# ShreyasBhaktharam/RDEIC

Hardware: AMD Instinct MI355X
Metric: 512x512 images/sec encode+relay-decode @ fixed bpp; 1/2/4/8 GPU (higher is better)
Workload: dtype bf16; 1 GPU; config 2: global batch 16 (16/GPU) 512x512, 2-step relay DDIM, encode+entropy-code+decode+VAE-decode; global_batch=16, image_size=512, ddim_steps=2, sampler=ddim, parallelism=dp1, codec_sessions_per_gpu=5

## Files before the change

include/rdeic_hip.h:

```cpp
#ifndef RDEIC_HIP_H
#define RDEIC_HIP_H
#include <stddef.h>
#include <stdint.h>
#ifdef __cplusplus
extern "C" {
#endif

int rdeic_version(void);
int rdeic_abi_count(void);

typedef struct rdeic_conv_desc {
  const void* in0;
  const void* in1;
  int32_t c0, c1;
  int32_t ld0, ld1;
  int32_t n, h, w;
  int32_t up2;
  const void* weight;
  int32_t wld;
  const float* bias;
  int32_t cout, kh, kw, stride, pad_t, pad_l;
  int32_t ho, wo;
  const float* gn_ab;
  int32_t gn_silu;
  const float* emb;
  int32_t emb_ld;
  int32_t act;
  float act_param;
  const void* res;
  int32_t res_ld;
  void* out;
  int32_t out_ld;
  int32_t out_mode;
  int32_t dtype;
  int32_t out_f32;
  int32_t batch;
  int64_t in_bs, w_bs, out_bs;
  float* gn_part;
  int32_t gn_hw;
  int32_t reserved;
  const float* ln_rows;
  const float* ln_colsum;
} rdeic_conv_desc;

int rdeic_conv2d(const rdeic_conv_desc* d, void* stream);
int rdeic_conv2d_tile(const rdeic_conv_desc* d, int32_t tile, void* stream);
int rdeic_conv2d_splitk(const rdeic_conv_desc* d, int32_t splits, float* ws, size_t ws_floats, void* stream);
int rdeic_conv2d_up2_phases(const rdeic_conv_desc* d, int64_t phase_stride, int32_t tile, void* stream);
int rdeic_conv2d_up2_group(const rdeic_conv_desc* d);
int rdeic_set_conv_path(int32_t path);
int rdeic_set_conv_option(int32_t key, int32_t value);

size_t rdeic_groupnorm_ws_floats(int32_t n, int32_t hw, int32_t c);
size_t rdeic_groupnorm_parts_floats(int64_t rows, int32_t c, int32_t hw);
int rdeic_groupnorm_parts_ab(const float* p0, int32_t c0, const float* p1, int32_t c1, int32_t n, int32_t hw,
// ... 104 lines not shown
#define RDEIC_PROF_GN_STATS 3
#define RDEIC_PROF_GN_APPLY 4
#define RDEIC_PROF_GEMM 5
#define RDEIC_PROF_ATTN_D512 6
#define RDEIC_PROF_CONV_BYTES 7
int rdeic_prof_start(int32_t capacity, int32_t every);
int rdeic_prof_read_keys(int32_t kind, int64_t* keys, int64_t* launches, double* work, double* ms, int32_t cap);
#define RDEIC_COUNT_HALO_CONV 0
#define RDEIC_COUNT_GN_APPLY 1
#define RDEIC_COUNT_LAYERNORM 2
#define RDEIC_COUNT_HALO_SMALL 3
#define RDEIC_COUNT_LN_FUSED 4
#define RDEIC_COUNT_SPLITK 5
#define RDEIC_COUNT_EDGE 6
#define RDEIC_COUNT_GN_PARTS_APPLY 7
#define RDEIC_COUNT_KINDS 8
int64_t rdeic_launch_count(int32_t kind);
int rdeic_layernorm_rowstats(const void* x, int32_t rows, int32_t c, int32_t ld, float eps, float* ms,
                             void* stream);
int rdeic_launch_count_reset(void);
int rdeic_prof_stop(void);
int rdeic_prof_read(int32_t kind, int64_t* launches, double* work, double* ms);

typedef struct rdeic_gemm_desc {
  const void* a;
  int64_t a_bs1, a_bs2, a_sm, a_sk;
  const void* b;
  int64_t b_bs1, b_bs2, b_sk, b_sn;
  void* c;
  int64_t c_bs1, c_bs2, c_sm;
  int32_t batch, nb2, m, n, k, ksplit, dtype, c_f32;
// ... 94 lines not shown
```

rdeic_amd/_lib.py:

```python
from __future__ import annotations

import ctypes as C
import os
import threading

_HERE = os.path.dirname(os.path.abspath(__file__))
LIB_PATH = os.environ.get("RDEIC_LIB") or os.path.join(_HERE, "lib", "librdeic_hip.so")

EINVAL, ENOSPC, EBADMSG, ELAUNCH = -22, -28, -74, -5
_ERRNAMES = {EINVAL: "EINVAL (bad argument/shape)", ENOSPC: "ENOSPC (output capacity)",
             EBADMSG: "EBADMSG (corrupt or truncated bitstream)", ELAUNCH: "kernel launch failure"}


class RdeicError(RuntimeError):
    def __init__(self, fn: str, code: int):
        super().__init__(f"{fn} failed: {code} {_ERRNAMES.get(code, '')}")
        self.code = code


class BitstreamError(RdeicError, ValueError):
    """Corrupt / truncated bitstream (the reference's 'decode failure')."""


class ConvDesc(C.Structure):
# ... 1 lines not shown
        ("in0", C.c_void_p), ("in1", C.c_void_p),
        ("c0", C.c_int32), ("c1", C.c_int32), ("ld0", C.c_int32), ("ld1", C.c_int32),
        ("n", C.c_int32), ("h", C.c_int32), ("w", C.c_int32), ("up2", C.c_int32),
        ("weight", C.c_void_p), ("wld", C.c_int32),
        ("bias", C.c_void_p),
        ("cout", C.c_int32), ("kh", C.c_int32), ("kw", C.c_int32), ("stride", C.c_int32),
        ("pad_t", C.c_int32), ("pad_l", C.c_int32),
        ("ho", C.c_int32), ("wo", C.c_int32),
        ("gn_ab", C.c_void_p), ("gn_silu", C.c_int32),
        ("emb", C.c_void_p), ("emb_ld", C.c_int32),
        ("act", C.c_int32), ("act_param", C.c_float),
        ("res", C.c_void_p), ("res_ld", C.c_int32),
        ("out", C.c_void_p), ("out_ld", C.c_int32), ("out_mode", C.c_int32),
        ("dtype", C.c_int32), ("out_f32", C.c_int32),
        ("batch", C.c_int32), ("in_bs", C.c_int64), ("w_bs", C.c_int64), ("out_bs", C.c_int64),
        ("gn_part", C.c_void_p), ("gn_hw", C.c_int32), ("reserved", C.c_int32),
        ("ln_rows", C.c_void_p), ("ln_colsum", C.c_void_p),
    ]


class GemmDesc(C.Structure):
    _fields_ = [
        ("a", C.c_void_p), ("a_bs1", C.c_int64), ("a_bs2", C.c_int64), ("a_sm", C.c_int64), ("a_sk", C.c_int64),
        ("b", C.c_void_p), ("b_bs1", C.c_int64), ("b_bs2", C.c_int64), ("b_sk", C.c_int64), ("b_sn", C.c_int64),
        ("c", C.c_void_p), ("c_bs1", C.c_int64), ("c_bs2", C.c_int64), ("c_sm", C.c_int64),
        ("batch", C.c_int32), ("nb2", C.c_int32), ("m", C.c_int32), ("n", C.c_int32), ("k", C.c_int32),
        ("ksplit", C.c_int32), ("dtype", C.c_int32), ("c_f32", C.c_int32),
        ("alpha", C.c_float), ("beta", C.c_float), ("rsum", C.c_void_p), ("rsum_bs", C.c_int64),
    ]


# ... 170 lines not shown
```

rdeic_amd/csrc/conv_common.h:

```cpp
#pragma once
#include "common.h"
#include "../../include/rdeic_hip.h"
#include "prof.h"

namespace rdeic_conv {

struct ConvArgs {
  const char* in0; const char* in1;
  int c0, c1, ld0, ld1;
  int n, h, w, up2;
  const char* weight; int wld;
  const float* bias;
  int cout, kh, kw, stride, pad_t, pad_l, ho, wo;
  const float* gn_ab; int gn_silu;
  const float* emb; int emb_ld;
  int act; float act_param;
  const char* res; int res_ld;
  char* out; int out_ld, out_mode;
  int out_f32;
  int M, cin, ktot, nk;
  long in_bs, w_bs, out_bs;
  int batch;
  int epi_vec;
  int splits, kper;
  float* gn_part;
  int gn_row0;
  int gn_hw;
  const float* ln_rows;
  const float* ln_cs;
};

__device__ __forceinline__ float ln_fold(const ConvArgs& a, int m, int n, float v) {
  const float2 ms = reinterpret_cast<const float2*>(a.ln_rows)[m];
  return ms.y * (v - ms.x * a.ln_cs[n]);
}

constexpr int ROWB = 144;

template <typename T, bool SWZ = true> __host__ __device__ constexpr int tile_rowb() { return (sizeof(T) == 2 && SWZ) ? 128 : ROWB; }
template <typename T, bool SWZ = true> __device__ __forceinline__ int chunk_key(int r) {
  if constexpr (sizeof(T) == 2 && SWZ) return (((r >> 3) & 1) << 1) | (((r >> 1) & 1) << 2);
  return 0;
}
template <typename T, int BM, int BN, bool SWZ = true> __host__ __device__ constexpr int conv_lds_bytes() {
// ... 395 lines not shown
      for (int h = 0; h < 2; ++h)
#pragma unroll
        for (int e = 0; e < 4; e += 2) {
          const f32x2 xv = {to_f32(from_f32<bf16>(v[8 * h + e])), to_f32(from_f32<bf16>(v[8 * h + e + 1]))};
          const f32x2 gt = {to_f32(from_f32<bf16>(v[8 * h + 4 + e])), to_f32(from_f32<bf16>(v[8 * h + 5 + e]))};
          const f32x2 r = xv * gelu_fast2(gt);
          gv[4 * h + e] = from_f32<bf16>(r.x);
          gv[4 * h + e + 1] = from_f32<bf16>(r.y);
        }
      *reinterpret_cast<uint4*>(reinterpret_cast<bf16*>(a.out) + (long)m * a.out_ld + (nn >> 1)) =
          *reinterpret_cast<uint4*>(gv);
    }
  }
}

constexpr unsigned kOOB = 0x80000000u;

template <int N>
__device__ __forceinline__ void wait_vm() {
  asm volatile("s_waitcnt vmcnt(%0)" ::"n"(N) : "memory");
}

__device__ __forceinline__ int dma_key(int r) { return (((r >> 3) & 1) << 1) | (((r >> 1) & 1) << 2); }

typedef __attribute__((address_space(3))) void* lds_ptr_t;

__device__ __forceinline__ void dma16(__amdgpu_buffer_rsrc_t rs, char* lds_dst, unsigned voff, int soff) {
  __builtin_amdgcn_raw_ptr_buffer_load_lds(rs, (lds_ptr_t)lds_dst, 16, (int)voff, soff, 0, 0);
}

// ... 8 lines not shown
#endif

__device__ __forceinline__ void wait_vm_rt(int n) {
  switch (n) {
    case 0: wait_vm<0>(); break;
    case 1: wait_vm<1>(); break;
    case 2: wait_vm<2>(); break;
    case 3: wait_vm<3>(); break;
    case 4: wait_vm<4>(); break;
    case 5: wait_vm<5>(); break;
    case 6: wait_vm<6>(); break;
    default: wait_vm<7>(); break;
  }
}

extern int g_conv_path, g_epi_vec, g_swz, g_force_tile, g_dma, g_halo, g_halo8, g_edge, g_up2_phases;

int make_args(const rdeic_conv_desc* d, ConvArgs& a, bool& vec);
bool dma_ok(const rdeic_conv_desc* d, const ConvArgs& a, unsigned& b0, unsigned& b1, unsigned& bw);
int launch_dma_auto(const ConvArgs& a, unsigned b0, unsigned b1, unsigned bw, hipStream_t s, int tile,
                    int gn_hw = 0, bool* fused = nullptr);
int dma_grouped(const rdeic_conv_desc* d, int tile, hipStream_t s, bool* fused = nullptr);
bool halo_ok(const rdeic_conv_desc* d, const ConvArgs& a);
int launch_halo(const rdeic_conv_desc* d, ConvArgs a, hipStream_t s, bool* fused);
int launch_edge(const rdeic_conv_desc* d, const ConvArgs& a, hipStream_t s, bool* fused);
int up2_phase_group(const rdeic_conv_desc* d);
bool up2_phases_ok(const rdeic_conv_desc* d, long phase_stride);
int launch_up2_phases(const rdeic_conv_desc* d, long phase_stride, int tile, hipStream_t s, bool* fused);
}
```

rdeic_amd/csrc/conv_dma.hip:

```cpp
#include "conv_common.h"

namespace rdeic_conv {

template <int TM, int TN, int WTM, int WTN, class PixMap = PixSame>
__device__ __forceinline__ void epilogue_scalar(const f32x4 (&acc)[TM][TN], const ConvArgs& a, int m0, int n0, int wm,
                                                int wn, int lane, PixMap pmap = PixMap{}) {
  if (a.out_mode == 2) return;
  const int lrow = lane & 15, lq = lane >> 4;
  const int hw_o = a.ho * a.wo;
  const bool of32 = a.out_f32;
#pragma unroll
  for (int i = 0; i < TM; ++i) {
#pragma unroll
    for (int r = 0; r < 4; ++r) {
      const int m = m0 + wm * WTM + i * 16 + lq * 4 + r;
      if (m >= a.M) continue;
      const int img = m / hw_o;
      int oy = 0, ox = 0;
      if (a.out_mode == 1) { const int rem = m - img * hw_o; oy = rem / a.wo; ox = rem - oy * a.wo; }
#pragma unroll
      for (int j = 0; j < TN; ++j) {
        const int nn = n0 + wn * WTN + j * 16 + lrow;
        if (nn >= a.cout) continue;
        float v = acc[i][j][r];
// ... 7 lines not shown
          const long p = ((long)img * (2 * a.ho) + (2 * oy + dy)) * (2 * a.wo) + (2 * ox + dx);
          oidx = p * a.out_ld + c;
          ridx = p * a.res_ld + c;
        } else {
          oidx = pmap(m) * a.out_ld + nn;
          ridx = pmap(m) * a.res_ld + nn;
        }
        if (a.res) v += of32 ? reinterpret_cast<const float*>(a.res)[ridx] : to_f32(reinterpret_cast<const bf16*>(a.res)[ridx]);
        if (of32) reinterpret_cast<float*>(a.out)[oidx] = v;
        else reinterpret_cast<bf16*>(a.out)[oidx] = from_f32<bf16>(v);
      }
    }
  }
}

template <int BM, int BN, int WGM, int WGN, int S, int EP, bool GEG = false, bool PH = false>
__device__ __forceinline__ void conv_dma_body(ConvArgs a, int tiles_n, unsigned bytes0, unsigned bytes1,
                                              unsigned bytesw) {
  constexpr int KB = 64;
  constexpr int NW = WGM * WGN, NT = NW * 64;
  constexpr int RB = KB * 2;
  constexpr int RPI = 1024 / RB;
  constexpr int LPR = RB / 16;
  constexpr int KSUB = KB / 32;
  constexpr int A_BYTES = BM * RB, STAGE = (BM + BN) * RB;
  constexpr int AI = BM / NW / RPI, BI = BN / NW / RPI;
  constexpr int PER = AI + BI;
  constexpr int WTM = BM / WGM, WTN = BN / WGN;
  constexpr int TM = WTM / 16, TN = WTN / 16;
  static_assert(AI >= 1 && BI >= 1 && AI * RPI * NW == BM && BI * RPI * NW == BN, "tile / wave split");
  static_assert(S >= 2 && S <= 4 && PER * (S - 2) <= 63, "ring");
// ... 159 lines not shown
  HALO_STAMP(2);
  if constexpr (PH) {
    const PixPhase pm{a.h, a.w, phase >> 1, phase & 1};
    if constexpr (TM % EP == 0 && (BM / EP) * (BN + 4) * 4 <= S * STAGE) {
      if (a.epi_vec && epi_vec_ok(a)) {
        epilogue_vec<BM, BN, WGM, WGN, NT, EP, RowsFrom, false, PixPhase>(acc, a, m0, n0, wm, wn, lane, tid, lds,
                                                                          RowsFrom{m0}, pm);
        HALO_STAMP(3);
        return;
      }
    }
    epilogue_scalar<TM, TN, WTM, WTN, PixPhase>(acc, a, m0, n0, wm, wn, lane, pm);
    HALO_STAMP(3);
    return;
  }
  if constexpr (TM % EP == 0 && (BM / EP) * (BN + 4) * 4 <= S * STAGE) {
    if ((a.epi_vec || a.out_mode == 2) && epi_vec_ok(a)) {
      if constexpr (GEG) epilogue_geglu<BM, BN, WGM, WGN, NT, EP>(acc, a, m0, n0, wm, wn, lane, tid, lds);
      else epilogue_vec<BM, BN, WGM, WGN, NT, EP>(acc, a, m0, n0, wm, wn, lane, tid, lds);
      HALO_STAMP(3);
      return;
    }
  }
  epilogue_scalar<TM, TN, WTM, WTN>(acc, a, m0, n0, wm, wn, lane);
  HALO_STAMP(3);
}

template <int BM, int BN, int WGM, int WGN, int S, int EP, bool GEG = false, bool PH = false>
__global__ __launch_bounds__(WGM * WGN * 64) void conv_dma_kernel(ConvArgs a, int tiles_n, unsigned bytes0,
                                                                  unsigned bytes1, unsigned bytesw) {
  conv_dma_body<BM, BN, WGM, WGN, S, EP, GEG, PH>(a, tiles_n, bytes0, bytes1, bytesw);
}

template <int BM, int BN, int WGM, int WGN, int S, int EP, bool GEG = false>
__global__ __launch_bounds__(WGM * WGN * 64) __attribute__((amdgpu_num_sgpr(80))) void conv_dma_kernel_2pc(
    ConvArgs a, int tiles_n, unsigned bytes0, unsigned bytes1, unsigned bytesw) {
  conv_dma_body<BM, BN, WGM, WGN, S, EP, GEG>(a, tiles_n, bytes0, bytes1, bytesw);
}

bool dma_ok(const rdeic_conv_desc* d, const ConvArgs& a, unsigned& b0, unsigned& b1, unsigned& bw) {
  if (d->dtype != 1 || d->gn_ab || (d->c0 % 64) || (d->c1 % 64) || (d->ld0 % 8) || ((uintptr_t)d->in0 % 16)) return false;
  if (d->c1 && ((d->ld1 % 8) || ((uintptr_t)d->in1 % 16))) return false;
  if (d->wld % 64 || a.ktot % 64) return false;
  const long pix = (long)d->n * d->h * d->w;
  const long e0 = ((pix - 1) * d->ld0 + d->c0) * 2 + (a.batch - 1) * d->in_bs * 2;
  const long e1 = d->c1 ? ((pix - 1) * d->ld1 + d->c1) * 2 : 16;
  const long ew = (long)d->cout * d->wld * 2 + (a.batch - 1) * d->w_bs * 2;
  if (e0 >= (1l << 31) || e1 >= (1l << 31) || ew >= (1l << 31)) return false;
  if (a.batch > 1 && (d->in_bs % 8 || d->w_bs % 8)) return false;
// ... 11 lines not shown
  return fits && (a.epi_vec || a.out_mode == 2) && epi_vec_ok(a);
}

template <int BM, int BN, int WGM, int WGN, int S, int EP>
int launch_dma(ConvArgs a, unsigned b0, unsigned b1, unsigned bw, hipStream_t s, int gn_hw, bool* fused) {
  if (a.gn_part) {
    const bool ok = a.splits <= 1 && a.batch == 1 && a.out_mode == 0 && gn_hw > 0 && gn_hw % 64 == 0 &&
                    stats_tile_ok<BM, BN, WGM, WGM * WGN * 64, EP>() && dma_vec_epilogue<BM, BN, WGM, WGN, S, EP>(a);
    if (!ok) a.gn_part = nullptr;
    if (fused) *fused = ok;
  }
  const int tn = cdiv(a.cout, BN);
  const long tiles = (long)cdiv(a.M, BM) * tn;
  dim3 grid((unsigned)tiles, 1, a.splits > 1 ? a.splits : a.batch);
  constexpr int lds = S * (BM + BN) * 128;
  const bool geg = a.out_mode == 2 && a.cout % 16 == 0 && a.out_ld % 8 == 0 && ((uintptr_t)a.out % 16) == 0 &&
                   dma_vec_epilogue<BM, BN, WGM, WGN, S, EP>(a);
  if constexpr (WGM * WGN == 16 && lds <= 80 * 1024) {
    hipLaunchKernelGGL((conv_dma_kernel_2pc<BM, BN, WGM, WGN, S, EP>), grid, dim3(WGM * WGN * 64), lds, s, a, tn, b0,
                       b1, bw);
  } else {
    if (geg)
      hipLaunchKernelGGL((conv_dma_kernel<BM, BN, WGM, WGN, S, EP, true>), grid, dim3(WGM * WGN * 64), lds, s, a, tn,
                         b0, b1, bw);
    else
      hipLaunchKernelGGL((conv_dma_kernel<BM, BN, WGM, WGN, S, EP>), grid, dim3(WGM * WGN * 64), lds, s, a, tn, b0, b1,
                         bw);
  }
  return launch_status();
}
}

int launch_dma_auto(const ConvArgs& a, unsigned b0, unsigned b1, unsigned bw, hipStream_t s, int tile, int gn_hw,
                    bool* fused) {
  if (tile < 21 || tile > 38) {
    const long zb = a.splits > 1 ? a.splits : a.batch;
    const long t128 = (long)cdiv(a.M, 128) * cdiv(a.cout, 128) * zb;
    const long t256 = (long)cdiv(a.M, 256) * cdiv(a.cout, 256) * zb;
// ... 56 lines not shown
  return RDEIC_OK;
}

namespace {
template <int BM, int BN, int WGM, int WGN, int S, int EP>
int launch_dma_ph(ConvArgs a, unsigned b0, unsigned b1, unsigned bw, hipStream_t s, bool* fused) {
  if (a.gn_part) {
    const bool ok = (a.h * a.w) % 64 == 0 && stats_tile_ok<BM, BN, WGM, WGM * WGN * 64, EP>() &&
                    dma_vec_epilogue<BM, BN, WGM, WGN, S, EP>(a);
    if (!ok) a.gn_part = nullptr;
    if (fused) *fused = ok;
  }
  const int tn = cdiv(a.cout, BN);
  const long tiles = (long)cdiv(a.M, BM) * 4 * tn;
  constexpr int lds = S * (BM + BN) * 128;
  hipLaunchKernelGGL((conv_dma_kernel<BM, BN, WGM, WGN, S, EP, false, true>), dim3((unsigned)tiles),
                     dim3(WGM * WGN * 64), lds, s, a, tn, b0, b1, bw);
  return launch_status();
}

int launch_ph_auto(const ConvArgs& a, unsigned b0, unsigned b1, unsigned bw, hipStream_t s, int tile, bool* fused) {
  if (tile != 32 && tile != 33 && tile != 25 && tile != 26 && tile != 30 && tile != 36) {
    const long t128 = (long)cdiv(a.M, 128) * cdiv(a.cout, 128) * 4;
    const long t256 = (long)cdiv(a.M, 256) * cdiv(a.cout, 256) * 4;
    const float useful256 = (float)a.M * a.cout / ((float)cdiv(a.M, 256) * 256 * cdiv(a.cout, 256) * 256);
    tile = (t256 >= 256 && useful256 >= 0.9f) ? 32 : t128 >= 256 ? 25 : 26;
  }
  switch (tile) {
    case 32: return launch_dma_ph<256, 256, 4, 4, 2, 4>(a, b0, b1, bw, s, fused);
    case 33: return launch_dma_ph<256, 128, 4, 4, 2, 2>(a, b0, b1, bw, s, fused);
    case 25: return launch_dma_ph<128, 128, 2, 4, 2, 2>(a, b0, b1, bw, s, fused);
// ... 60 lines not shown
```

rdeic_amd/csrc/conv_gemm.hip:

```cpp
#include "conv_common.h"

namespace rdeic_conv {

int g_conv_path = 2;
int g_epi_vec = 1;
int g_swz = 1;
int g_force_tile = -1;
int g_dma = 1;
int g_halo = 1;
int g_halo8 = 1;
int g_up2_phases = 1;

namespace {

template <typename T, int BM, int BN, int WGM, int WGN, bool VEC, bool GNP = true, bool SWZ = true>
__global__ __launch_bounds__(WGM * WGN * 64) void conv_kernel(ConvArgs a) {
  constexpr int NT = WGM * WGN * 64;
  constexpr int BK = MmaTraits<T>::BK;
  constexpr int EPC = MmaTraits<T>::EPC;
  constexpr int ES = sizeof(T);
  constexpr int WTM = BM / WGM, WTN = BN / WGN;
  constexpr int TM = WTM / 16, TN = WTN / 16;
  constexpr int RPI = NT / 8;
  constexpr int AR = BM / RPI;
  constexpr int BR = (BN + RPI - 1) / RPI;
  static_assert(TM >= 1 && TN >= 1 && AR >= 1 && BM % RPI == 0, "tile");
// ... 480 lines not shown
    return RDEIC_EINVAL;
  a.M = d->n * d->ho * d->wo;
  a.batch = d->batch > 1 ? d->batch : 1;
  a.in_bs = d->in_bs; a.w_bs = d->w_bs; a.out_bs = d->out_bs;
  if (a.batch > 1 && (d->res || d->emb || d->out_mode)) return RDEIC_EINVAL;
  a.cin = d->c0 + d->c1;
  a.ktot = d->kh * d->kw * a.cin;
  const int BK = d->dtype == 1 ? 64 : 32;
  if (d->wld < a.ktot || d->wld % 64 != 0) return RDEIC_EINVAL;
  a.nk = (a.ktot + BK - 1) / BK;
  if (d->out_mode < 0 || d->out_mode > 2) return RDEIC_EINVAL;
  if (d->out_mode == 1 && (d->cout % 4 != 0)) return RDEIC_EINVAL;
  if (d->out_mode == 2 && (d->dtype != 1 || d->cout % 8 || d->res || d->emb || d->act || d->out_f32 || d->gn_ab ||
                           a.batch > 1 || d->out_ld % 4 || ((uintptr_t)d->out) % 8))
    return RDEIC_EINVAL;
  const int epc = d->dtype == 1 ? 8 : 4;
  vec = (d->c0 % epc == 0) && (d->ld0 % epc == 0) && (((uintptr_t)d->in0) % 16 == 0);
  if (d->c1) vec = vec && (d->c1 % epc == 0) && (d->ld1 % epc == 0) && (((uintptr_t)d->in1) % 16 == 0);
  if (((uintptr_t)d->weight) % 16 != 0) return RDEIC_EINVAL;
  return RDEIC_OK;
}
}

using namespace rdeic_conv;

static int conv2d_run(const rdeic_conv_desc* d, void* stream, bool* fused) {
  ConvArgs a;
  bool vec = false;
  const int rc = make_args(d, a, vec);
  if (rc != RDEIC_OK) return rc;
// ... 213 lines not shown

extern int rdeic_g_attn64;
extern int rdeic_g_attn512;

extern "C" int rdeic_set_conv_option(int32_t key, int32_t value) {
  if (key == 0) { int prev = g_epi_vec; g_epi_vec = value; return prev; }
  if (key == 1) { int prev = rdeic_g_attn64; rdeic_g_attn64 = value; return prev; }
  if (key == 3) { int prev = g_swz; g_swz = value; return prev; }
  if (key == 4) { int prev = g_force_tile; g_force_tile = value; return prev; }
  if (key == 5) { int prev = g_dma; g_dma = value; return prev; }
  if (key == 6) { int prev = g_halo; g_halo = value; return prev; }
  if (key == 8) { int prev = rdeic_g_attn512; rdeic_g_attn512 = value; return prev; }
  if (key == 9) { int prev = g_halo8; g_halo8 = value; return prev; }
  if (key == 10) { int prev = g_edge; g_edge = value; return prev; }
  if (key == 11) { int prev = g_up2_phases; g_up2_phases = value; return prev; }
  return RDEIC_EINVAL;
}
```

rdeic_amd/ops.py:

```python
from __future__ import annotations

import ctypes as C
import json
import math
import os
import threading
from dataclasses import dataclass
from typing import Optional

import torch

from . import _lib
from ._lib import ConvDesc, call

NONE, LEAKY, GELU, SILU = 0, 1, 2, 3


def dt_code(t: torch.Tensor) -> int:
    if t.dtype == torch.bfloat16:
        return 1
    if t.dtype == torch.float32:
        return 0
    raise TypeError(f"unsupported activation dtype {t.dtype}")

# ... 21 lines not shown
    return torch.empty((n, h, w, c), dtype=dtype, device=device or "cuda")


@dataclass
class ConvParams:
    weight: torch.Tensor
    wld: int
    bias: Optional[torch.Tensor]
    cout: int
    cin: int
    kh: int
    kw: int
    stride: int = 1
    pad: int = 0
    ln_cs: Optional[torch.Tensor] = None

    @staticmethod
    def pack(w: torch.Tensor, b: Optional[torch.Tensor], stride: int = 1, pad: int = 0,
             dtype=torch.bfloat16) -> "ConvParams":
        if w.dim() == 2:
            w = w[:, :, None, None]
        w = w.detach().to(device="cuda", dtype=torch.float32).contiguous()
        cout, cin, kh, kw = w.shape
        wld = ((kh * kw * cin + 63) // 64) * 64
        packed = torch.empty((cout, wld), dtype=dtype, device="cuda")
        call("rdeic_pack_conv_weight", w.data_ptr(), cout, cin, kh, kw, packed.data_ptr(), wld,
             1 if dtype == torch.bfloat16 else 0, stream_ptr())
        bias = None if b is None else b.detach().to(device="cuda", dtype=torch.float32).contiguous()
        return ConvParams(packed, wld, bias, cout, cin, kh, kw, stride, pad)

# ... 75 lines not shown
        d.gn_silu = int(gn_silu)
    if emb is not None:
        if emb.dtype != torch.float32 or emb.shape[0] != n or emb.stride(1) != 1:
            raise ValueError("emb must be fp32 [n, >=cout] row-major")
        d.emb = emb.data_ptr()
        d.emb_ld = emb.stride(0)
    d.act, d.act_param = act, float(slope)
    if res is not None:
        if tuple(res.shape) != oshape or res.dtype != odt:
            raise ValueError(f"residual {tuple(res.shape)}/{res.dtype} does not match output {oshape}/{odt}")
        d.res = res.data_ptr()
        d.res_ld = pix_ld(res)
    d.out = out.data_ptr()
    d.out_ld = pix_ld(out)
    d.out_mode = 2 if geglu else (1 if pixel_shuffle else 0)
    d.dtype = dt_code(x)
    d.out_f32 = int(odt == torch.float32 and x.dtype != torch.float32)
    d.batch = 1
    if ln_rows is not None:
        if p.ln_cs is None or ln_rows.dtype != torch.float32 or tuple(ln_rows.shape) != (n * ho * wo, 2) \
                or not ln_rows.is_contiguous():
            raise ValueError("ln_rows needs a ParamStore.conv_ln weight and an fp32 [M, 2] contiguous (mean, rstd)")
        d.ln_rows, d.ln_colsum = ln_rows.data_ptr(), p.ln_cs.data_ptr()
    elif p.ln_cs is not None:
        raise ValueError("a LayerNorm-folded weight needs ln_rows")
    part = None
    if stats and GN_STATS_FUSE and x.dtype == torch.bfloat16 and not (geglu or pixel_shuffle):
        ghw = int(stats_hw or ho * wo)
        nf = int(_lib.load().rdeic_groupnorm_parts_floats(n * ho * wo, p.cout, ghw))
        if nf:
# ... 1 lines not shown
            d.gn_part, d.gn_hw = part.data_ptr(), ghw
    flops = 2.0 * n * ho * wo * p.cout * p.kh * p.kw * p.cin
    splits = _splitk_count(x, x2, n * ho * wo, p, gn is not None or pixel_shuffle or geglu, out,
                           n if images is None else images)

    tile = -1
    if splits == 1 and x.dtype == torch.bfloat16 and gn is None and _gn_materialize(x, x2, p):
        key = tile_key(n * ho * wo, c0, c1, p, up2, d.out_mode, res is not None, emb is not None, act, odt)
        tile = TILE_TABLE.get(key, -1) if FORCE_TILE is None else FORCE_TILE
        if AUTOTUNE and FORCE_TILE is None and key not in TILE_TABLE:
            scratch = torch.empty_strided(out.size(), out.stride(), dtype=out.dtype, device=out.device)
            dma = c0 % 64 == 0 and c1 % 64 == 0
            tile = _autotune_tile(d, scratch, DMA_TILE_CANDIDATES if dma else TILE_CANDIDATES)
            if tile >= 0:
                TILE_TABLE[key] = tile

    if up2 and phases is not None and UP2_PHASES and splits == 1 and x.dtype == torch.bfloat16 and gn is None \
            and x2 is None and emb is None and res is None and ln_rows is None and d.out_mode == 0 and not d.out_f32 \
            and (p.kh, p.kw, p.stride, pt, pl) == (3, 3, 1, 1, 1) and (ho, wo) == (2 * h, 2 * w) \
            and phases.weight.dtype == torch.bfloat16 and phases.cout == p.cout and phases.wld == 4 * c0:
        dp = ConvDesc.from_buffer_copy(d)
        dp.weight, dp.wld = phases.weight.data_ptr(), phases.wld
        key = tile_key(n * h * w, c0, 0, phases, 2, 0, False, False, act, odt)
        ptile = TILE_TABLE.get(key, -1) if FORCE_TILE is None else FORCE_TILE
        ptag = ("conv", 2.0 * n * h * w * 4 * c0 * p.cout * 4,
                (n, h, w, c0, c1, p.cout, p.kh, p.stride, False, 2, d.out_mode))
        if _launch_soft(ptag, "rdeic_conv2d_up2_phases", C.byref(dp), phases.weight.stride(0), ptile, stream_ptr()):
            if part is not None:
                _attach_gn_part(out, part, d.gn_hw)
            return out
# ... 19 lines not shown

def _gn_part_of(t: Optional[torch.Tensor], hw: int):
    info = getattr(t, "_rdeic_gn_part", None) if t is not None else None
    if info is None:
        return None
    part, ptr, shape, stride, phw = info
    if ptr != t.data_ptr() or shape != tuple(t.shape) or stride != tuple(t.stride()) or phw != hw:
        return None
    return part


AUTOTUNE = False
UP2_PHASES = True
FORCE_TILE: Optional[int] = None
GEGLU_FUSED = True
TILE_CANDIDATES = (0, 1, 3, 4, 6, 8, 10)
DMA_TILE_CANDIDATES = (25, 32, 34, 26, 30, 33, 24, 31, 35, 36, 37, 38)
ALL_TILES = (0, 1, 2, 3, 4, 6, 7, 8, 9, 10) + tuple(range(21, 39))
TILE_TABLE_PATH = os.environ.get("RDEIC_TILE_TABLE") or os.path.join(os.path.dirname(os.path.abspath(__file__)),
                                                                     "conv_tiles.json")


def tile_key(m: int, c0: int, c1: int, p: "ConvParams", up2, out_mode: int, res: bool, emb: bool, act: int,
             odt) -> str:
    return (f"m{m}:c{c0}+{c1}:o{p.cout}:k{p.kh}x{p.kw}:s{p.stride}:up{int(up2)}:om{out_mode}:"
            f"r{int(res)}:e{int(emb)}:a{act}:{'f32' if odt == torch.float32 else 'bf16'}")


def _load_tile_table() -> dict:
    if not os.path.exists(TILE_TABLE_PATH):
        return {}
    with open(TILE_TABLE_PATH) as f:
        tab = json.load(f)["tiles"]
    bad = {k: v for k, v in tab.items() if v not in ALL_TILES}
    if bad:
        raise ValueError(f"{TILE_TABLE_PATH}: unknown tile ids {bad}")
    return tab


TILE_TABLE: dict = _load_tile_table()

# ... 203 lines not shown
    return out


CONV_PATH = 2


def set_conv_path(path: int) -> int:
    global CONV_PATH
    prev = CONV_PATH
    CONV_PATH = int(path)
    _lib.load().rdeic_set_conv_path(CONV_PATH)
    return prev


def set_conv_option(key: int, value: int) -> int:
    return int(_lib.load().rdeic_set_conv_option(int(key), int(value)))


HALO_CONV = 1
HALO_MAX_C = 512


COUNT_HALO_CONV, COUNT_GN_APPLY, COUNT_LAYERNORM, COUNT_HALO_SMALL, COUNT_LN_FUSED, COUNT_SPLITK, COUNT_EDGE, \
    COUNT_GN_PARTS_APPLY = 0, 1, 2, 3, 4, 5, 6, 7


def set_up2_phases(on: bool) -> bool:
    global UP2_PHASES
    prev = UP2_PHASES
    UP2_PHASES = bool(on)
    _lib.load().rdeic_set_conv_option(11, int(UP2_PHASES))
    return prev


def launch_count(kind: int) -> int:
    return int(_lib.load().rdeic_launch_count(int(kind)))


def launch_count_reset() -> None:
# ... 284 lines not shown
```

rdeic_amd/params.py:

```python
from __future__ import annotations

from typing import Dict, Iterable, Optional, Sequence, Tuple

import torch

from . import ops
from . import weights as W


def fold_up2_phases(w: torch.Tensor, dtype=torch.float32) -> torch.Tensor:
    cout, cin, kh, kw = w.shape
    if (kh, kw) != (3, 3):
        raise ValueError("the phase fold is for 3x3 convs")
    r = torch.tensor([[[1, 0, 0], [0, 1, 1]], [[1, 1, 0], [0, 0, 1]]], dtype=torch.float64, device=w.device)
    f = torch.einsum("ayk,oikl,bxl->aboyxi", r, w.double(), r)
    return f.reshape(4, cout, 4 * cin).to(dtype).contiguous()


class ParamStore:
    def __init__(self, compute_dtype=torch.bfloat16, device="cuda"):
        self.compute_dtype = compute_dtype
        self.device = torch.device(device)
        self.shapes: Dict[str, Tuple[int, ...]] = {}
        self.t: Dict[str, torch.Tensor] = {}
        self._packed: Dict[tuple, ops.ConvParams] = {}

    def declare(self, name: str, shape: Sequence[int]):
        shape = tuple(int(s) for s in shape)
        if name in self.shapes and self.shapes[name] != shape:
            raise ValueError(f"{name} declared twice with different shapes")
        self.shapes[name] = shape
# ... 79 lines not shown

    def conv_split_pad(self, prefix: str, c0: int, c0_pad: int, dtype=None) -> ops.ConvParams:
        dtype = dtype or self.compute_dtype
        key = (prefix, "split_pad", c0, c0_pad, dtype)
        p = self._packed.get(key)
        if p is None:
            w = self.t[prefix + ".weight"]
            cout, cin, kh, kw = w.shape
            wp = torch.zeros((cout, cin - c0 + c0_pad, kh, kw), dtype=w.dtype, device=w.device)
            wp[:, :c0] = w[:, :c0]
            wp[:, c0_pad:] = w[:, c0:]
            p = ops.ConvParams.pack(wp, self.t.get(prefix + ".bias"), stride=1, pad=kh // 2, dtype=dtype)
            self._packed[key] = p
        return p

    def conv_geglu(self, prefix: str, dtype=None) -> ops.ConvParams:
        dtype = dtype or self.compute_dtype
        key = (prefix, "geglu", dtype)
        p = self._packed.get(key)
        if p is None:
            w = self.t[prefix + ".weight"]
            b = self.t.get(prefix + ".bias")
            c = w.shape[0] // 2
            if c % 4:
                raise ValueError("GEGLU width must be a multiple of 4")
            perm = torch.arange(2 * c, device=w.device).view(2, c // 4, 4).permute(1, 0, 2).reshape(-1)
            p = ops.ConvParams.pack(w[perm], None if b is None else b[perm], dtype=dtype)
            self._packed[key] = p
        return p

    def conv_ln(self, prefixes: Sequence[str], ln_prefix: str, geglu: bool = False, dtype=None) -> ops.ConvParams:
        dtype = dtype or self.compute_dtype
        key = (tuple(prefixes), "ln", ln_prefix, geglu, dtype)
        p = self._packed.get(key)
        if p is None:
            gamma, beta = self.t[ln_prefix + ".weight"], self.t[ln_prefix + ".bias"]
            ws, bs = [], []
            for pre in prefixes:
                w = self.t[pre + ".weight"]
                b = self.t.get(pre + ".bias")
                ws.append(w)
                bs.append(b if b is not None else torch.zeros(w.shape[0], device=self.device))
            w = torch.cat(ws, 0)
            b = torch.cat(bs, 0).double() + w.double() @ beta.double()
            w = w * gamma[None, :]
            if geglu:
                c = w.shape[0] // 2
                perm = torch.arange(2 * c, device=w.device).view(2, c // 4, 4).permute(1, 0, 2).reshape(-1)
                w, b = w[perm], b[perm]
            p = ops.ConvParams.pack(w, b.float(), dtype=dtype)
            p.ln_cs = p.weight.double().sum(1).float().contiguous()
            self._packed[key] = p
        return p

    def conv_cat(self, prefixes: Sequence[str], dtype=None) -> ops.ConvParams:
        dtype = dtype or self.compute_dtype
        key = (tuple(prefixes), "cat", dtype)
        p = self._packed.get(key)
        if p is None:
            ws, bs = [], []
            for pre in prefixes:
                w = self.t[pre + ".weight"]
                ws.append(w if w.dim() == 4 else w[:, :, None, None])
                b = self.t.get(pre + ".bias")
                bs.append(b if b is not None else torch.zeros(w.shape[0], device=self.device))
            any_bias = any(self.t.get(pre + ".bias") is not None for pre in prefixes)
# ... 6 lines not shown
```

rdeic_amd/unet.py:

```python
from __future__ import annotations

from dataclasses import dataclass, field
from typing import List, Optional

import torch

from . import ops
from .params import ParamStore


def find_denominator(number: int, start: int) -> int:
    if start >= number:
        return number
    while start != 0:
        if number % start == 0:
            return start
        start -= 1
    return 1


@dataclass
class ResBlock:
    prefix: str
    cin: int
# ... 186 lines not shown
        o = torch.empty((rows, C), dtype=x.dtype, device=x.device)
        ops.attention(qkv[:, :C], qkv[:, C:2 * C], qkv[:, 2 * C:], o, batch=B, heads=t.heads, lq=L, lk=L, dh=t.dh,
                      scale=scale)
        h = ops.linear(o, s.conv(tb + ".attn1.to_out.0"), res=h, images=B)
        if fold:
            q = ops.linear(h, s.conv_ln([tb + ".attn2.to_q"], tb + ".norm2"), ln_rows=ops.layer_norm_rowstats(h),
                           images=B)
        else:
            n2 = ops.layer_norm(h, s.get(tb + ".norm2.weight"), s.get(tb + ".norm2.bias"))
            q = ops.linear(n2, s.conv(tb + ".attn2.to_q"), images=B)
        kv = ops.linear(ctx_kv_in, s.conv_cat([tb + ".attn2.to_k", tb + ".attn2.to_v"]), images=ctx_batch)
        ops.attention(q, kv[:, :C], kv[:, C:], o, batch=B, heads=t.heads, lq=L, lk=ctx_len, dh=t.dh, scale=scale,
                      kv_bcast=(ctx_batch == 1 and B > 1))
        h = ops.linear(o, s.conv(tb + ".attn2.to_out.0"), res=h, images=B)
        if fold and ops.GEGLU_FUSED:
            gg = ops.linear(h, s.conv_ln([tb + ".ff.net.0.proj"], tb + ".norm3", geglu=True),
                            ln_rows=ops.layer_norm_rowstats(h), geglu=True, images=B)
        else:
            n3 = ops.layer_norm(h, s.get(tb + ".norm3.weight"), s.get(tb + ".norm3.bias"))
            if x.dtype == torch.bfloat16 and ops.GEGLU_FUSED and C % 64 == 0:
                gg = ops.linear(n3, s.conv_geglu(tb + ".ff.net.0.proj"), geglu=True, images=B)
            else:
                gg = ops.geglu(ops.linear(n3, s.conv(tb + ".ff.net.0.proj"), images=B))
        h = ops.linear(gg, s.conv(tb + ".ff.net.2"), res=h, images=B)
        if not x.is_contiguous():
            raise ValueError("transformer input must be contiguous NHWC")
        out = ops.linear(h, s.conv(t.prefix + ".proj_out"), res=x.view(rows, C), stats_hw=L if stats else None,
                         images=B)
        return ops.tokens_to_nhwc(out, B, H, W_)

    def run_layers(self, layers, x, emb_all, ctx_rows, ctx_batch, ctx_len, x2=None, stats_last: bool = True):
        s = self.store
        for li, layer in enumerate(layers):
            st = stats_last or li + 1 < len(layers)
            if isinstance(layer, Conv):
                x = ops.conv2d(x, s.conv(layer.prefix), x2=x2, stats=st)
# ... 129 lines not shown
```

Baseline: 161.4 images/s.

## Compute GEGLU in registers by interleaving value/gate weights at 16-column granularity

Adds a new GEGLU epilogue for the DMA conv/GEMM kernel that pairs value and gate accumulator fragments directly in registers. The fused FF projection weights are permuted into 16-wide value/gate groups to make this possible, and the epilogue writes bf16 results to LDS in a swizzled layout before coalesced stores. This is meant to replace the previous epilogue that staged fp32 tiles through LDS before applying GEGLU, cutting LDS traffic and barriers. It adds a new weight-packing layout, a host flag and option key, and excludes certain tiles where the layout does not fit.

```diff
diff --git a/include/rdeic_hip.h b/include/rdeic_hip.h
--- a/include/rdeic_hip.h
+++ b/include/rdeic_hip.h
@@ -38,7 +38,7 @@
   int64_t in_bs, w_bs, out_bs;
   float* gn_part;
   int32_t gn_hw;
-  int32_t reserved;
+  int32_t geglu_layout;
   const float* ln_rows;
   const float* ln_colsum;
 } rdeic_conv_desc;
@@ -173,7 +173,8 @@
 #define RDEIC_COUNT_SPLITK 5
 #define RDEIC_COUNT_EDGE 6
 #define RDEIC_COUNT_GN_PARTS_APPLY 7
-#define RDEIC_COUNT_KINDS 8
+#define RDEIC_COUNT_GEGLU_REGS 8
+#define RDEIC_COUNT_KINDS 9
 int64_t rdeic_launch_count(int32_t kind);
 int rdeic_layernorm_rowstats(const void* x, int32_t rows, int32_t c, int32_t ld, float eps, float* ms,
                              void* stream);
diff --git a/rdeic_amd/_lib.py b/rdeic_amd/_lib.py
--- a/rdeic_amd/_lib.py
+++ b/rdeic_amd/_lib.py
@@ -39,7 +39,7 @@
         ("out", C.c_void_p), ("out_ld", C.c_int32), ("out_mode", C.c_int32),
         ("dtype", C.c_int32), ("out_f32", C.c_int32),
         ("batch", C.c_int32), ("in_bs", C.c_int64), ("w_bs", C.c_int64), ("out_bs", C.c_int64),
-        ("gn_part", C.c_void_p), ("gn_hw", C.c_int32), ("reserved", C.c_int32),
+        ("gn_part", C.c_void_p), ("gn_hw", C.c_int32), ("geglu_layout", C.c_int32),
         ("ln_rows", C.c_void_p), ("ln_colsum", C.c_void_p),
     ]
 
diff --git a/rdeic_amd/csrc/conv_common.h b/rdeic_amd/csrc/conv_common.h
--- a/rdeic_amd/csrc/conv_common.h
+++ b/rdeic_amd/csrc/conv_common.h
@@ -28,6 +28,7 @@
   int gn_hw;
   const float* ln_rows;
   const float* ln_cs;
+  int geg_regs;
 };
 
 __device__ __forceinline__ float ln_fold(const ConvArgs& a, int m, int n, float v) {
@@ -453,6 +454,97 @@
   }
 }
 
+template <int BM, int BN, int WGM, int WGN, int S>
+__host__ __device__ constexpr bool geglu_regs_tile_ok() {
+  constexpr int TN = BN / WGN / 16, CPR = BN / 16;
+  return TN % 2 == 0 && BN % 32 == 0 && CPR >= 4 && (CPR & (CPR - 1)) == 0 && WGM * WGN * 64 >= BM &&
+         BM * BN + BM * 8 <= S * (BM + BN) * 128;
+}
+
+template <int BM, int BN, int WGM, int WGN, int NT, int P>
+__device__ __forceinline__ void epilogue_geglu_regs(const f32x4 (&acc)[BM / WGM / 16][BN / WGN / 16],
+                                                    const ConvArgs& a, int m0, int n0, int wm, int wn, int lane,
+                                                    int tid, char* lds) {
+  constexpr int WTM = BM / WGM, WTN = BN / WGN;
+  constexpr int TM = WTM / 16, TN = WTN / 16, TQ = TN / 2;
+  constexpr int HM = TM / P;
+  constexpr int PR = BM / P;
+  constexpr int RBY = BN;
+  constexpr int CPR = BN / 16;
+  constexpr int NCH = (PR * CPR + NT - 1) / NT;
+  static_assert(TM % P == 0 && TN % 2 == 0 && NT >= BM, "P passes, value / gate fragment pairs, one thread per row");
+  typedef bf16 bf16x2 __attribute__((ext_vector_type(2)));
+  const int lr = lane & 15, lq = lane >> 4;
+  float* ST = reinterpret_cast<float*>(lds + BM * RBY);
+  auto bar = []() { asm volatile("s_waitcnt lgkmcnt(0)\n\ts_barrier" ::: "memory"); };
+  const bool ln = a.ln_rows != nullptr;
+  float2 st = float2{0.f, 0.f};
+  if (ln && tid < BM && m0 + tid < a.M) st = reinterpret_cast<const float2*>(a.ln_rows)[m0 + tid];
+  float bs[TN], cs[TN];
+#pragma unroll
+  for (int j = 0; j < TN; ++j) {
+    const int nn = n0 + wn * WTN + j * 16 + lr;
+    bs[j] = (a.bias && nn < a.cout) ? a.bias[nn] : -0.f;
+    cs[j] = (ln && nn < a.cout) ? a.ln_cs[nn] : 0.f;
+  }
+  bar();
+  if (ln) {
+    if (tid < BM) reinterpret_cast<float2*>(ST)[tid] = st;
+    bar();
+  }
+  const int key = (lq & 1) << 1;
+#pragma unroll
+  for (int p = 0; p < P; ++p) {
+    char* R = lds + p * PR * RBY;
+#pragma unroll
+    for (int ii = 0; ii < HM; ++ii) {
+      const int i = p * HM + ii;
+      float mr[4] = {0.f, 0.f, 0.f, 0.f}, rr[4] = {1.f, 1.f, 1.f, 1.f};
+      if (ln) {
+        const float* sp = ST + (wm * WTM + i * 16 + lq * 4) * 2;
+        const float4 s0 = *reinterpret_cast<const float4*>(sp), s1 = *reinterpret_cast<const float4*>(sp + 4);
+        mr[0] = s0.x; rr[0] = s0.y; mr[1] = s0.z; rr[1] = s0.w;
+        mr[2] = s1.x; rr[2] = s1.y; mr[3] = s1.z; rr[3] = s1.w;
+      }
+#pragma unroll
+      for (int r = 0; r < 4; r += 2) {
+        const f32x2 nm = {-mr[r], -mr[r + 1]}, rs = {rr[r], rr[r + 1]};
+        char* Rr = R + (wm * (WTM / P) + ii * 16 + lq * 4 + r) * RBY;
+#pragma unroll
+        for (int q = 0; q < TQ; ++q) {
+#pragma clang fp contract(off)
+          f32x2 xv = {acc[i][2 * q][r], acc[i][2 * q][r + 1]};
+          f32x2 gt = {acc[i][2 * q + 1][r], acc[i][2 * q + 1][r + 1]};
+          xv = rs * pk_fma(nm, f32x2{cs[2 * q], cs[2 * q]}, xv);
+          gt = rs * pk_fma(nm, f32x2{cs[2 * q + 1], cs[2 * q + 1]}, gt);
+          xv = xv + f32x2{bs[2 * q], bs[2 * q]};
+          gt = gt + f32x2{bs[2 * q + 1], bs[2 * q + 1]};
+          xv = __builtin_convertvector(__builtin_convertvector(xv, bf16x2), f32x2);
+          gt = __builtin_convertvector(__builtin_convertvector(gt, bf16x2), f32x2);
+          const bf16x2 o = __builtin_convertvector(xv * gelu_fast2(gt), bf16x2);
+          const int oc = wn * (WTN / 2) + q * 16 + lr;
+          const int off = (((oc >> 3) ^ key) << 4) + (oc & 7) * 2;
+          *reinterpret_cast<bf16*>(Rr + off) = o.x;
+          *reinterpret_cast<bf16*>(Rr + RBY + off) = o.y;
+        }
+      }
+    }
+    bar();
+#pragma unroll
+    for (int k = 0; k < NCH; ++k) {
+      const int c = tid + k * NT;
+      if (c >= PR * CPR) continue;
+      const int pr = c / CPR, cc = c - pr * CPR;
+      const int wmr = pr / (WTM / P), wr = pr - wmr * (WTM / P);
+      const int m = m0 + wmr * WTM + p * (WTM / P) + wr;
+      const int oc = (n0 >> 1) + cc * 8;
+      if (m >= a.M || oc >= (a.cout >> 1)) continue;
+      const uint4 v = *reinterpret_cast<const uint4*>(R + pr * RBY + ((cc ^ (((pr >> 2) & 1) << 1)) << 4));
+      *reinterpret_cast<uint4*>(reinterpret_cast<bf16*>(a.out) + (long)m * a.out_ld + oc) = v;
+    }
+  }
+}
+
 constexpr unsigned kOOB = 0x80000000u;
 
 template <int N>
@@ -491,7 +583,7 @@
   }
 }
 
-extern int g_conv_path, g_epi_vec, g_swz, g_force_tile, g_dma, g_halo, g_halo8, g_edge, g_up2_phases;
+extern int g_conv_path, g_epi_vec, g_swz, g_force_tile, g_dma, g_halo, g_halo8, g_edge, g_up2_phases, g_geglu_regs;
 
 int make_args(const rdeic_conv_desc* d, ConvArgs& a, bool& vec);
 bool dma_ok(const rdeic_conv_desc* d, const ConvArgs& a, unsigned& b0, unsigned& b1, unsigned& bw);
diff --git a/rdeic_amd/csrc/conv_dma.hip b/rdeic_amd/csrc/conv_dma.hip
--- a/rdeic_amd/csrc/conv_dma.hip
+++ b/rdeic_amd/csrc/conv_dma.hip
@@ -45,7 +45,7 @@
   }
 }
 
-template <int BM, int BN, int WGM, int WGN, int S, int EP, bool GEG = false, bool PH = false>
+template <int BM, int BN, int WGM, int WGN, int S, int EP, int GEG = 0, bool PH = false>
 __device__ __forceinline__ void conv_dma_body(ConvArgs a, int tiles_n, unsigned bytes0, unsigned bytes1,
                                               unsigned bytesw) {
   constexpr int KB = 64;
@@ -235,9 +235,14 @@
     HALO_STAMP(3);
     return;
   }
+  if constexpr (GEG == 2) {
+    epilogue_geglu_regs<BM, BN, WGM, WGN, NT, EP>(acc, a, m0, n0, wm, wn, lane, tid, lds);
+    HALO_STAMP(3);
+    return;
+  }
   if constexpr (TM % EP == 0 && (BM / EP) * (BN + 4) * 4 <= S * STAGE) {
     if ((a.epi_vec || a.out_mode == 2) && epi_vec_ok(a)) {
-      if constexpr (GEG) epilogue_geglu<BM, BN, WGM, WGN, NT, EP>(acc, a, m0, n0, wm, wn, lane, tid, lds);
+      if constexpr (GEG == 1) epilogue_geglu<BM, BN, WGM, WGN, NT, EP>(acc, a, m0, n0, wm, wn, lane, tid, lds);
       else epilogue_vec<BM, BN, WGM, WGN, NT, EP>(acc, a, m0, n0, wm, wn, lane, tid, lds);
       HALO_STAMP(3);
       return;
@@ -247,13 +252,13 @@
   HALO_STAMP(3);
 }
 
-template <int BM, int BN, int WGM, int WGN, int S, int EP, bool GEG = false, bool PH = false>
+template <int BM, int BN, int WGM, int WGN, int S, int EP, int GEG = 0, bool PH = false>
 __global__ __launch_bounds__(WGM * WGN * 64) void conv_dma_kernel(ConvArgs a, int tiles_n, unsigned bytes0,
                                                                   unsigned bytes1, unsigned bytesw) {
   conv_dma_body<BM, BN, WGM, WGN, S, EP, GEG, PH>(a, tiles_n, bytes0, bytes1, bytesw);
 }
 
-template <int BM, int BN, int WGM, int WGN, int S, int EP, bool GEG = false>
+template <int BM, int BN, int WGM, int WGN, int S, int EP, int GEG = 0>
 __global__ __launch_bounds__(WGM * WGN * 64) __attribute__((amdgpu_num_sgpr(80))) void conv_dma_kernel_2pc(
     ConvArgs a, int tiles_n, unsigned bytes0, unsigned bytes1, unsigned bytesw) {
   conv_dma_body<BM, BN, WGM, WGN, S, EP, GEG>(a, tiles_n, bytes0, bytes1, bytesw);
@@ -295,6 +300,20 @@
   const long tiles = (long)cdiv(a.M, BM) * tn;
   dim3 grid((unsigned)tiles, 1, a.splits > 1 ? a.splits : a.batch);
   constexpr int lds = S * (BM + BN) * 128;
+  if (a.geg_regs) {
+    constexpr bool tile_ok = geglu_regs_tile_ok<BM, BN, WGM, WGN, S>() && (BM / WGM / 16) % EP == 0 &&
+                             !(WGM * WGN == 16 && lds <= 80 * 1024);
+    if constexpr (tile_ok) {
+      if (a.out_mode != 2 || a.cout % 32 || a.out_ld % 8 || ((uintptr_t)a.out % 16) || a.splits > 1 || a.batch > 1)
+        return RDEIC_EINVAL;
+      hipLaunchKernelGGL((conv_dma_kernel<BM, BN, WGM, WGN, S, EP, 2>), grid, dim3(WGM * WGN * 64), lds, s, a, tn, b0,
+                         b1, bw);
+      rdeic_count_launch(RDEIC_COUNT_GEGLU_REGS);
+      return launch_status();
+    } else {
+      return RDEIC_EINVAL;
+    }
+  }
   const bool geg = a.out_mode == 2 && a.cout % 16 == 0 && a.out_ld % 8 == 0 && ((uintptr_t)a.out % 16) == 0 &&
                    dma_vec_epilogue<BM, BN, WGM, WGN, S, EP>(a);
   if constexpr (WGM * WGN == 16 && lds <= 80 * 1024) {
@@ -302,7 +321,7 @@
                        b1, bw);
   } else {
     if (geg)
-      hipLaunchKernelGGL((conv_dma_kernel<BM, BN, WGM, WGN, S, EP, true>), grid, dim3(WGM * WGN * 64), lds, s, a, tn,
+      hipLaunchKernelGGL((conv_dma_kernel<BM, BN, WGM, WGN, S, EP, 1>), grid, dim3(WGM * WGN * 64), lds, s, a, tn,
                          b0, b1, bw);
     else
       hipLaunchKernelGGL((conv_dma_kernel<BM, BN, WGM, WGN, S, EP>), grid, dim3(WGM * WGN * 64), lds, s, a, tn, b0, b1,
@@ -389,7 +408,7 @@
   const int tn = cdiv(a.cout, BN);
   const long tiles = (long)cdiv(a.M, BM) * 4 * tn;
   constexpr int lds = S * (BM + BN) * 128;
-  hipLaunchKernelGGL((conv_dma_kernel<BM, BN, WGM, WGN, S, EP, false, true>), dim3((unsigned)tiles),
+  hipLaunchKernelGGL((conv_dma_kernel<BM, BN, WGM, WGN, S, EP, 0, true>), dim3((unsigned)tiles),
                      dim3(WGM * WGN * 64), lds, s, a, tn, b0, b1, bw);
   return launch_status();
 }
diff --git a/rdeic_amd/csrc/conv_gemm.hip b/rdeic_amd/csrc/conv_gemm.hip
--- a/rdeic_amd/csrc/conv_gemm.hip
+++ b/rdeic_amd/csrc/conv_gemm.hip
@@ -10,6 +10,7 @@
 int g_halo = 1;
 int g_halo8 = 1;
 int g_up2_phases = 1;
+int g_geglu_regs = 1;
 
 namespace {
 
@@ -520,6 +521,10 @@
   if (d->out_mode == 2 && (d->dtype != 1 || d->cout % 8 || d->res || d->emb || d->act || d->out_f32 || d->gn_ab ||
                            a.batch > 1 || d->out_ld % 4 || ((uintptr_t)d->out) % 8))
     return RDEIC_EINVAL;
+  if (d->geglu_layout != 0 && (d->geglu_layout != 1 || d->out_mode != 2 || !g_geglu_regs || !g_dma || d->cout % 32 ||
+                               d->out_ld % 8 || ((uintptr_t)d->out) % 16))
+    return RDEIC_EINVAL;
+  a.geg_regs = d->geglu_layout == 1;
   const int epc = d->dtype == 1 ? 8 : 4;
   vec = (d->c0 % epc == 0) && (d->ld0 % epc == 0) && (((uintptr_t)d->in0) % 16 == 0);
   if (d->c1) vec = vec && (d->c1 % epc == 0) && (d->ld1 % epc == 0) && (((uintptr_t)d->in1) % 16 == 0);
@@ -763,5 +768,6 @@
   if (key == 9) { int prev = g_halo8; g_halo8 = value; return prev; }
   if (key == 10) { int prev = g_edge; g_edge = value; return prev; }
   if (key == 11) { int prev = g_up2_phases; g_up2_phases = value; return prev; }
+  if (key == 13) { int prev = g_geglu_regs; g_geglu_regs = value; return prev; }
   return RDEIC_EINVAL;
 }
diff --git a/rdeic_amd/ops.py b/rdeic_amd/ops.py
--- a/rdeic_amd/ops.py
+++ b/rdeic_amd/ops.py
@@ -59,6 +59,7 @@
     stride: int = 1
     pad: int = 0
     ln_cs: Optional[torch.Tensor] = None
+    geglu_layout: int = 0
 
     @staticmethod
     def pack(w: torch.Tensor, b: Optional[torch.Tensor], stride: int = 1, pad: int = 0,
@@ -164,6 +165,9 @@
     d.out = out.data_ptr()
     d.out_ld = pix_ld(out)
     d.out_mode = 2 if geglu else (1 if pixel_shuffle else 0)
+    if p.geglu_layout and not geglu:
+        raise ValueError("a GEGLU-packed weight of layout 1 runs with geglu=True only")
+    d.geglu_layout = p.geglu_layout if geglu else 0
     d.dtype = dt_code(x)
     d.out_f32 = int(odt == torch.float32 and x.dtype != torch.float32)
     d.batch = 1
@@ -195,6 +199,8 @@
             tile = _autotune_tile(d, scratch, DMA_TILE_CANDIDATES if dma else TILE_CANDIDATES)
             if tile >= 0:
                 TILE_TABLE[key] = tile
+    if d.geglu_layout == 1 and tile in GEGLU_REGS_EXCLUDED_TILES:
+        tile = -1
 
     if up2 and phases is not None and UP2_PHASES and splits == 1 and x.dtype == torch.bfloat16 and gn is None \
             and x2 is None and emb is None and res is None and ln_rows is None and d.out_mode == 0 and not d.out_f32 \
@@ -244,6 +250,8 @@
 UP2_PHASES = True
 FORCE_TILE: Optional[int] = None
 GEGLU_FUSED = True
+GEGLU_REGS = True
+GEGLU_REGS_EXCLUDED_TILES = (34, 37, 38)
 TILE_CANDIDATES = (0, 1, 3, 4, 6, 8, 10)
 DMA_TILE_CANDIDATES = (25, 32, 34, 26, 30, 33, 24, 31, 35, 36, 37, 38)
 ALL_TILES = (0, 1, 2, 3, 4, 6, 7, 8, 9, 10) + tuple(range(21, 39))
@@ -255,6 +263,15 @@
              odt) -> str:
     return (f"m{m}:c{c0}+{c1}:o{p.cout}:k{p.kh}x{p.kw}:s{p.stride}:up{int(up2)}:om{out_mode}:"
             f"r{int(res)}:e{int(emb)}:a{act}:{'f32' if odt == torch.float32 else 'bf16'}")
+
+
+def geglu_layout(rows: int, cin: int, cout: int) -> int:
+    if not GEGLU_REGS or AUTOTUNE or cout % 32 or cin % 64:
+        return 0
+    tile = FORCE_TILE
+    if tile is None:
+        tile = TILE_TABLE.get(f"m{rows}:c{cin}+0:o{cout}:k1x1:s1:up0:om2:r0:e0:a0:bf16", -1)
+    return 0 if tile in GEGLU_REGS_EXCLUDED_TILES else 1
 
 
 def _load_tile_table() -> dict:
@@ -488,7 +505,16 @@
 
 
 def set_conv_option(key: int, value: int) -> int:
+    global GEGLU_REGS
+    if int(key) == 13:
+        GEGLU_REGS = bool(value)
     return int(_lib.load().rdeic_set_conv_option(int(key), int(value)))
+
+
+def set_geglu_regs(on: bool) -> bool:
+    prev = GEGLU_REGS
+    set_conv_option(13, int(bool(on)))
+    return prev
 
 
 HALO_CONV = 1
@@ -496,7 +522,7 @@
 
 
 COUNT_HALO_CONV, COUNT_GN_APPLY, COUNT_LAYERNORM, COUNT_HALO_SMALL, COUNT_LN_FUSED, COUNT_SPLITK, COUNT_EDGE, \
-    COUNT_GN_PARTS_APPLY = 0, 1, 2, 3, 4, 5, 6, 7
+    COUNT_GN_PARTS_APPLY, COUNT_GEGLU_REGS = 0, 1, 2, 3, 4, 5, 6, 7, 8
 
 
 def set_up2_phases(on: bool) -> bool:
diff --git a/rdeic_amd/params.py b/rdeic_amd/params.py
--- a/rdeic_amd/params.py
+++ b/rdeic_amd/params.py
@@ -15,6 +15,20 @@
     r = torch.tensor([[[1, 0, 0], [0, 1, 1]], [[1, 1, 0], [0, 0, 1]]], dtype=torch.float64, device=w.device)
     f = torch.einsum("ayk,oikl,bxl->aboyxi", r, w.double(), r)
     return f.reshape(4, cout, 4 * cin).to(dtype).contiguous()
+
+
+def geglu_perm(c: int, layout: int = 0, device=None) -> Tuple[torch.Tensor, int]:
+    g = 16 if (layout == 1 and c % 16 == 0) else 4
+    if c % g:
+        raise ValueError("GEGLU width must be a multiple of 4")
+    perm = torch.arange(2 * c, device=device).view(2, c // g, g).permute(1, 0, 2).reshape(-1)
+    return perm, int(g == 16)
+
+
+def fold_layernorm(w: torch.Tensor, b: Optional[torch.Tensor], gamma: torch.Tensor,
+                   beta: torch.Tensor) -> Tuple[torch.Tensor, torch.Tensor]:
+    b0 = b.double() if b is not None else torch.zeros(w.shape[0], dtype=torch.float64, device=w.device)
+    return w * gamma[None, :], b0 + w.double() @ beta.double()
 
 
 class ParamStore:
@@ -124,24 +138,28 @@
             self._packed[key] = p
         return p
 
-    def conv_geglu(self, prefix: str, dtype=None) -> ops.ConvParams:
+    def conv_geglu(self, prefix: str, dtype=None, layout: int = 0) -> ops.ConvParams:
         dtype = dtype or self.compute_dtype
-        key = (prefix, "geglu", dtype)
+        w = self.t[prefix + ".weight"]
+        perm, layout = geglu_perm(w.shape[0] // 2, layout, w.device)
+        key = (prefix, "geglu", dtype, layout)
         p = self._packed.get(key)
         if p is None:
-            w = self.t[prefix + ".weight"]
             b = self.t.get(prefix + ".bias")
-            c = w.shape[0] // 2
-            if c % 4:
-                raise ValueError("GEGLU width must be a multiple of 4")
-            perm = torch.arange(2 * c, device=w.device).view(2, c // 4, 4).permute(1, 0, 2).reshape(-1)
             p = ops.ConvParams.pack(w[perm], None if b is None else b[perm], dtype=dtype)
+            p.geglu_layout = layout
             self._packed[key] = p
         return p
 
-    def conv_ln(self, prefixes: Sequence[str], ln_prefix: str, geglu: bool = False, dtype=None) -> ops.ConvParams:
+    def conv_ln(self, prefixes: Sequence[str], ln_prefix: str, geglu: bool = False, dtype=None,
+                layout: int = 0) -> ops.ConvParams:
         dtype = dtype or self.compute_dtype
-        key = (tuple(prefixes), "ln", ln_prefix, geglu, dtype)
+        if geglu:
+            perm, layout = geglu_perm(sum(self.t[pre + ".weight"].shape[0] for pre in prefixes) // 2, layout,
+                                      self.device)
+        else:
+            layout = 0
+        key = (tuple(prefixes), "ln", ln_prefix, geglu, dtype, layout)
         p = self._packed.get(key)
         if p is None:
             gamma, beta = self.t[ln_prefix + ".weight"], self.t[ln_prefix + ".bias"]
@@ -151,15 +169,12 @@
                 b = self.t.get(pre + ".bias")
                 ws.append(w)
                 bs.append(b if b is not None else torch.zeros(w.shape[0], device=self.device))
-            w = torch.cat(ws, 0)
-            b = torch.cat(bs, 0).double() + w.double() @ beta.double()
-            w = w * gamma[None, :]
+            w, b = fold_layernorm(torch.cat(ws, 0), torch.cat(bs, 0), gamma, beta)
             if geglu:
-                c = w.shape[0] // 2
-                perm = torch.arange(2 * c, device=w.device).view(2, c // 4, 4).permute(1, 0, 2).reshape(-1)
                 w, b = w[perm], b[perm]
             p = ops.ConvParams.pack(w, b.float(), dtype=dtype)
             p.ln_cs = p.weight.double().sum(1).float().contiguous()
+            p.geglu_layout = layout
             self._packed[key] = p
         return p
 
diff --git a/rdeic_amd/unet.py b/rdeic_amd/unet.py
--- a/rdeic_amd/unet.py
+++ b/rdeic_amd/unet.py
@@ -224,12 +224,14 @@
                       kv_bcast=(ctx_batch == 1 and B > 1))
         h = ops.linear(o, s.conv(tb + ".attn2.to_out.0"), res=h, images=B)
         if fold and ops.GEGLU_FUSED:
-            gg = ops.linear(h, s.conv_ln([tb + ".ff.net.0.proj"], tb + ".norm3", geglu=True),
+            gg = ops.linear(h, s.conv_ln([tb + ".ff.net.0.proj"], tb + ".norm3", geglu=True,
+                                         layout=ops.geglu_layout(rows, C, 8 * C)),
                             ln_rows=ops.layer_norm_rowstats(h), geglu=True, images=B)
         else:
             n3 = ops.layer_norm(h, s.get(tb + ".norm3.weight"), s.get(tb + ".norm3.bias"))
             if x.dtype == torch.bfloat16 and ops.GEGLU_FUSED and C % 64 == 0:
-                gg = ops.linear(n3, s.conv_geglu(tb + ".ff.net.0.proj"), geglu=True, images=B)
+                gg = ops.linear(n3, s.conv_geglu(tb + ".ff.net.0.proj", layout=ops.geglu_layout(rows, C, 8 * C)),
+                                geglu=True, images=B)
             else:
                 gg = ops.geglu(ops.linear(n3, s.conv(tb + ".ff.net.0.proj"), images=B))
         h = ops.linear(gg, s.conv(tb + ".ff.net.2"), res=h, images=B)
```

Result: no change. 161.6 images/s, median of 2 (+0.1%).
